# zkh2018/ethsnarks

Measured on AMD Instinct MI355X. Metric: groth16_proofs_per_sec, higher is better.
Workload: dtype u32 (8-limb 254-bit Montgomery integers)

## Files before the change

ethsnarks_amd/csrc/ntt.hpp:

```cpp
#pragma once
#include "bn254.hpp"
#include "common.hpp"

namespace zk {

#ifndef ZK_NTT_TILE_LOG
#define ZK_NTT_TILE_LOG 11
#endif
constexpr int NTT_TILE_LOG = ZK_NTT_TILE_LOG;
constexpr int NTT_TILE = 1 << NTT_TILE_LOG;
#ifndef ZK_NTT_THREADS
#define ZK_NTT_THREADS 512
#endif
constexpr int NTT_THREADS = ZK_NTT_THREADS;
constexpr int NTT_MIN_LOGC = 2;

static ZK_HD uint32_t bitrev32(uint32_t v, uint32_t bits) {
#if defined(__clang__)
    return bits ? __builtin_bitreverse32(v) >> (32 - bits) : 0;
#else
    uint32_t r = 0;
    for (uint32_t i = 0; i < bits; i++) { r = (r << 1) | (v & 1); v >>= 1; }
    return r;
#endif
}

struct NttFuse { const fe *in2 = nullptr; const fe *post_alt = nullptr; uint32_t alt_from = 0xffffffffu; const fe *sub = nullptr; };
__global__ void __launch_bounds__(NTT_THREADS)
k_ntt_pass(const fe *__restrict__ in, fe *__restrict__ out, const fe *__restrict__ tw,
           uint32_t logm, uint32_t s0, uint32_t k, uint32_t logc, int bitrev_load,
           const fe *__restrict__ pre, const fe *__restrict__ post, uint32_t batch_stride, NttFuse fuse, int last_pass) {
    __shared__ uint32_t sh[8][NTT_TILE];
    in += (size_t)blockIdx.y * batch_stride; out += (size_t)blockIdx.y * batch_stride;
    if (fuse.in2) fuse.in2 += (size_t)blockIdx.y * batch_stride;
    if (fuse.sub) fuse.sub += (size_t)blockIdx.y * batch_stride;
    if (fuse.post_alt && blockIdx.y >= fuse.alt_from) post = fuse.post_alt;
    const uint32_t tile = 1u << (k + logc), ncol = 1u << logc;
    const uint32_t nlb = (1u << s0) >> logc;
    const uint32_t lb = blockIdx.x & (nlb - 1), h = blockIdx.x / nlb;
    const uint32_t base = (h << (s0 + k)) | (lb << logc);

    auto gidx = [&](uint32_t e) -> uint32_t { return base | ((e >> logc) << s0) | (e & (ncol - 1)); };
    auto fetch = [&](uint32_t idx) -> fe {
        const uint32_t src = bitrev_load ? bitrev32(idx, logm) : idx;
        fe v = in[src];
        if (fuse.in2) v = Fr::mul(v, fuse.in2[src]);
        if (pre) v = Fr::mul(v, pre[src]);
        return v;
    };
    auto emit = [&](uint32_t idx, fe v) {
        if (post) v = Fr::mul(v, post[idx]);
        else if (last_pass) v = Fr::canon(v);
        if (fuse.sub) v = Fr::sub(v, fuse.sub[idx]);
        out[idx] = v;
    };
    const bool load_fused = k >= 2;
    if (!load_fused) {
        for (uint32_t e = threadIdx.x; e < tile; e += blockDim.x) {
            const fe v = fetch(gidx(e));
#pragma unroll
            for (int l = 0; l < 8; l++) sh[l][e] = v.l[l];
        }
        __syncthreads();
    }
    uint32_t s = 1;
    for (; s + 1 <= k; s += 2) {
        const uint32_t half = 1u << (s - 1), S = s0 + s;
        const bool from_mem = s == 1, to_mem = s + 1 == k;
        for (uint32_t qd = threadIdx.x; qd < (tile >> 2); qd += blockDim.x) {
            const uint32_t c = qd & (ncol - 1), r = qd >> logc;
            const uint32_t jm = r & (half - 1), grp = r >> (s - 1);
            const uint32_t e00 = (((grp << (s + 1)) | jm) << logc) | c, e01 = e00 + (half << logc), e10 = e00 + (half << (logc + 1)), e11 = e10 + (half << logc);
            const uint32_t j = (jm << s0) | ((lb << logc) | c);
            const size_t i2 = (size_t)j << (logm - S - 1);
            fe x0, x1, x2, x3;
            if (from_mem) { x0 = fetch(gidx(e00)); x1 = fetch(gidx(e01)); x2 = fetch(gidx(e10)); x3 = fetch(gidx(e11)); }
            else {
#pragma unroll
                for (int l = 0; l < 8; l++) { x0.l[l] = sh[l][e00]; x1.l[l] = sh[l][e01]; x2.l[l] = sh[l][e10]; x3.l[l] = sh[l][e11]; }
            }
#ifdef ZK_NTT_NOPAIR
            if (S > 1) { const fe t1 = tw[i2 << 1]; x1 = Fr::lmul(x1, t1); x3 = Fr::lmul(x3, t1); }
#else
            if (S > 1) { const fe t1 = tw[i2 << 1]; Fr::lmul_pair(x1, t1, x3, t1, x1, x3); }
#endif
            fe a0 = Fr::ladd(x0, x1), a1 = Fr::lsub(x0, x1), a2 = Fr::ladd(x2, x3), a3 = Fr::lsub(x2, x3);
            if (S == 1) a3 = Fr::lmul(a3, tw[(size_t)1 << (logm - 2)]);
            else {
#ifdef ZK_NTT_NOPAIR
                a2 = Fr::lmul(a2, tw[i2]); a3 = Fr::lmul(a3, tw[i2 + ((size_t)1 << (logm - 2))]);
#else
                Fr::lmul_pair(a2, tw[i2], a3, tw[i2 + ((size_t)1 << (logm - 2))], a2, a3);
#endif
            }
            x0 = Fr::ladd(a0, a2); x2 = Fr::lsub(a0, a2); x1 = Fr::ladd(a1, a3); x3 = Fr::lsub(a1, a3);
            if (to_mem) { emit(gidx(e00), x0); emit(gidx(e01), x1); emit(gidx(e10), x2); emit(gidx(e11), x3); }
            else {
#pragma unroll
                for (int l = 0; l < 8; l++) { sh[l][e00] = x0.l[l]; sh[l][e01] = x1.l[l]; sh[l][e10] = x2.l[l]; sh[l][e11] = x3.l[l]; }
            }
        }
        if (!to_mem) __syncthreads();
    }
    if (s <= k) {
        const uint32_t half = 1u << (s - 1), S = s0 + s;
        for (uint32_t bf = threadIdx.x; bf < (tile >> 1); bf += blockDim.x) {
            uint32_t c = bf & (ncol - 1), q = bf >> logc;
            uint32_t jm = q & (half - 1), grp = q >> (s - 1);
            uint32_t eu = (((grp << s) | jm) << logc) | c, ev = eu + (half << logc);
            uint32_t j = (jm << s0) | ((lb << logc) | c);
            fe u, v;
#pragma unroll
            for (int l = 0; l < 8; l++) { u.l[l] = sh[l][eu]; v.l[l] = sh[l][ev]; }
            if (S > 1) v = Fr::lmul(v, tw[(size_t)j << (logm - S)]);
            emit(gidx(eu), Fr::ladd(u, v)); emit(gidx(ev), Fr::lsub(u, v));
        }
    } else if (k == 0) {
        for (uint32_t e = threadIdx.x; e < tile; e += blockDim.x) {
            fe v;
#pragma unroll
            for (int l = 0; l < 8; l++) v.l[l] = sh[l][e];
            emit(gidx(e), v);
        }
    }
}

__global__ void k_fill_geometric(fe *out, uint32_t n, fe g, fe s) {
    uint32_t run = blockIdx.x * blockDim.x + threadIdx.x;
    uint32_t i0 = run * 256;
// ... 18 lines not shown
static inline fe fr_domain_root(uint32_t logm) {
    fe w; const uint32_t c[8] = {0x725b19f0u, 0x9bd61b6eu, 0x41112ed4u, 0x402d111eu, 0x8ef62abcu, 0x00e0a7ebu, 0xa58a7e85u, 0x2a3c09f0u};
    for (int i = 0; i < 8; i++) w.l[i] = c[i];
    w = Fr::to_mont(w);
    for (uint32_t i = logm; i < 28; i++) w = Fr::sqr(w);
    return w;
}

static inline int ntt_tables_free(NttTables &t) {
    if (t.tw_fwd) hipFree(t.tw_fwd);
    if (t.tw_inv) hipFree(t.tw_inv);
    if (t.coset_fwd) hipFree(t.coset_fwd);
    if (t.inv_m) hipFree(t.inv_m);
    if (t.icoset) hipFree(t.icoset);
    if (t.inv_then_coset) hipFree(t.inv_then_coset);
    if (t.inv_m_zinv) hipFree(t.inv_m_zinv);
    if (t.icoset_zinv) hipFree(t.icoset_zinv);
    t = NttTables();
    return ZK_OK;
}

static inline int ntt_tables_create(NttTables &t, uint32_t logm, hipStream_t st) {
    if (logm > 28) return ZK_ERR_ARG;
    t.logm = logm;
    const uint32_t m = 1u << logm, half = m > 1 ? m / 2 : 1;
    ZK_HIP(hipMalloc(&t.tw_fwd, sizeof(fe) * half));
    ZK_HIP(hipMalloc(&t.tw_inv, sizeof(fe) * half));
    ZK_HIP(hipMalloc(&t.coset_fwd, sizeof(fe) * m));
    ZK_HIP(hipMalloc(&t.inv_m, sizeof(fe) * m));
    ZK_HIP(hipMalloc(&t.icoset, sizeof(fe) * m));
    ZK_HIP(hipMalloc(&t.inv_then_coset, sizeof(fe) * m));
    ZK_HIP(hipMalloc(&t.inv_m_zinv, sizeof(fe) * m));
    ZK_HIP(hipMalloc(&t.icoset_zinv, sizeof(fe) * m));
    const fe w = fr_domain_root(logm), wi = Fr::inv(w), g = Fr::from_u64(5), gi = Fr::inv(g);
    const fe mi = Fr::inv(Fr::from_u64(m)), one = Fr::one();
    t.zinv = Fr::inv(Fr::sub(Fr::pow_u64(g, m), one));
    auto fill = [&](fe *dst, uint32_t n, const fe &base, const fe &scale) {
        uint32_t runs = zk_div_up(n, 256);
        ZK_LAUNCH(k_fill_geometric, zk_div_up(runs, 64), 64, st, dst, n, base, scale);
    };
    fill(t.tw_fwd, half, w, one);
    fill(t.tw_inv, half, wi, one);
    fill(t.coset_fwd, m, g, one);
    fill(t.inv_m, m, one, mi);
    fill(t.icoset, m, gi, mi);
    fill(t.inv_then_coset, m, g, mi);
    fill(t.inv_m_zinv, m, one, Fr::mul(mi, t.zinv));
    fill(t.icoset_zinv, m, gi, Fr::mul(mi, t.zinv));
    ZK_HIP(hipGetLastError());
    return ZK_OK;
}

static inline int ntt_run(const NttTables &t, const fe *in, fe *out, bool inverse,
                          const fe *pre, const fe *post, hipStream_t st, uint32_t batch = 1, uint32_t stride = 0, NttFuse fuse = NttFuse()) {
    const uint32_t logm = t.logm, m = 1u << logm;
    const fe *tw = inverse ? t.tw_inv : t.tw_fwd;
    if (logm == 0) {
        uint32_t k0 = 0;
        ZK_LAUNCH_SYNC(k_ntt_pass, dim3(1, batch), NTT_THREADS, st, in, out, tw, logm, 0u, k0, 0u, 1, pre, post, stride, fuse, 1);
        return ZK_OK;
    }
    const uint32_t k0 = logm < (uint32_t)NTT_TILE_LOG ? logm : NTT_TILE_LOG;
    uint32_t rem = logm - k0;
    const uint32_t kmax = NTT_TILE_LOG - NTT_MIN_LOGC;
    uint32_t npass = (rem + kmax - 1) / kmax;
    NttFuse first = fuse, later = fuse;
    later.in2 = nullptr;
    if (rem != 0) { first.post_alt = nullptr; first.sub = nullptr; }
    ZK_LAUNCH_SYNC(k_ntt_pass, dim3(m >> k0, batch), NTT_THREADS, st, in, out, tw, logm, 0u, k0, 0u, 1, pre,
                   rem == 0 ? post : (const fe *)nullptr, stride, first, rem == 0 ? 1 : 0);
    uint32_t s0 = k0;
    while (rem) {
        uint32_t k = (rem + npass - 1) / npass;
        uint32_t logc = NTT_TILE_LOG - k;
        if (logc > s0) logc = s0;
        rem -= k; npass--;
        NttFuse f = later;
        if (rem != 0) { f.post_alt = nullptr; f.sub = nullptr; }
        ZK_LAUNCH_SYNC(k_ntt_pass, dim3(m >> (k + logc), batch), NTT_THREADS, st, (const fe *)out, out, tw, logm, s0, k, logc, 0,
                       (const fe *)nullptr, rem == 0 ? post : (const fe *)nullptr, stride, f, rem == 0 ? 1 : 0);
        s0 += k;
    }
    ZK_HIP(hipGetLastError());
    return ZK_OK;
}

constexpr uint32_t SPMV_LONG_ROW = 64;
constexpr uint32_t SPMV_CHUNK = 4096;

static ZK_HD bool fr_is_one(const fe &a) {
    uint32_t t = 0;
#pragma unroll
    for (int i = 0; i < 8; i++) t |= a.l[i] ^ FrParams::one(i);
    return t == 0;
}
static ZK_D fe spmv_term(const fe &coef, const fe &x) { return fr_is_one(coef) ? x : Fr::mul(coef, x); }

__global__ void k_spmv_rows(const uint32_t *__restrict__ row_ptr, const uint32_t *__restrict__ col,
                            const fe *__restrict__ coeff, const fe *__restrict__ w, fe *__restrict__ out, uint32_t n_rows,
                            uint32_t w_stride, uint32_t out_stride, uint32_t m_rows, uint32_t n_in_rows) {
    uint32_t j = blockIdx.x * blockDim.x + threadIdx.x;
    if (j >= m_rows) return;
    w += (size_t)blockIdx.y * w_stride; out += (size_t)blockIdx.y * out_stride;
    if (j >= n_rows) { out[j] = j - n_rows < n_in_rows ? w[j - n_rows] : Fr::zero(); return; }
    uint32_t b = row_ptr[j], e = row_ptr[j + 1];
    if (e - b > SPMV_LONG_ROW) return;
    fe acc = Fr::zero();
    for (uint32_t k = b; k < e; k++) acc = Fr::add(acc, spmv_term(coeff[k], w[col[k]]));
    out[j] = acc;
}

__global__ void __launch_bounds__(256)
k_spmv_long_chunks(const uint32_t *__restrict__ chunk_begin, const uint32_t *__restrict__ chunk_end,
                   const uint32_t *__restrict__ col, const fe *__restrict__ coeff, const fe *__restrict__ w,
                   fe *__restrict__ partial, uint32_t w_stride) {
    __shared__ uint32_t sh[8][256];
    w += (size_t)blockIdx.y * w_stride; partial += (size_t)blockIdx.y * gridDim.x;
    const uint32_t b = chunk_begin[blockIdx.x], e = chunk_end[blockIdx.x];
    fe acc = Fr::zero();
    for (uint32_t k = b + threadIdx.x; k < e; k += blockDim.x) acc = Fr::add(acc, spmv_term(coeff[k], w[col[k]]));
#pragma unroll
    for (int l = 0; l < 8; l++) sh[l][threadIdx.x] = acc.l[l];
    __syncthreads();
    for (uint32_t s = 128; s > 0; s >>= 1) {
        if (threadIdx.x < s) {
            fe o;
#pragma unroll
            for (int l = 0; l < 8; l++) o.l[l] = sh[l][threadIdx.x + s];
            acc = Fr::add(acc, o);
#pragma unroll
            for (int l = 0; l < 8; l++) sh[l][threadIdx.x] = acc.l[l];
        }
        __syncthreads();
    }
    if (threadIdx.x == 0) partial[blockIdx.x] = acc;
}

__global__ void __launch_bounds__(256)
k_spmv_long_finish(const uint32_t *__restrict__ long_row, const uint32_t *__restrict__ long_first_chunk,
                   const fe *__restrict__ partial, fe *__restrict__ out, uint32_t n_long, uint32_t n_chunks, uint32_t out_stride) {
    __shared__ uint32_t sh[8][256];
    const uint32_t i = blockIdx.x;
    if (i >= n_long) return;
    partial += (size_t)blockIdx.y * n_chunks; out += (size_t)blockIdx.y * out_stride;
    fe acc = Fr::zero();
    for (uint32_t k = long_first_chunk[i] + threadIdx.x; k < long_first_chunk[i + 1]; k += blockDim.x) acc = Fr::add(acc, partial[k]);
#pragma unroll
    for (int l = 0; l < 8; l++) sh[l][threadIdx.x] = acc.l[l];
    __syncthreads();
// ... 16 lines not shown
```

ethsnarks_amd/csrc/zkhip.cpp:

```cpp
#include <algorithm>
#include <atomic>
#include <memory>
#include <mutex>
#include <new>
#include <stdexcept>
#include <string>
#include <vector>
#include <chrono>
#include <string.h>
#include <stddef.h>
#include <stdlib.h>
#include <sys/stat.h>

#include "common.hpp"
#include "bn254.hpp"
#include "ntt.hpp"
#include "msm.hpp"
#include "keygen.hpp"
#include "blind.hpp"
#include "../../include/zkhip.h"
#include <errno.h>
#include <sys/random.h>

namespace zk { thread_local char g_last_error[256] = ""; }
// ... 448 lines not shown
    return full_save(path, codec, k);
} ZK_GUARD
extern "C" int zk_pk_is_full(const zk_pk *pk) try { return pk && pk->full ? 1 : 0; } ZK_GUARD

namespace {
struct DevCsr {
    uint32_t n_rows = 0, nnz = 0, n_long = 0, n_chunks = 0;
    uint32_t *row_ptr = nullptr, *col = nullptr, *long_row = nullptr, *long_first = nullptr, *chunk_begin = nullptr, *chunk_end = nullptr;
    fe *coeff = nullptr, *partial = nullptr;
    void release() {
        void *p[] = {row_ptr, col, long_row, long_first, chunk_begin, chunk_end, coeff, partial};
        for (void *q : p) if (q) hipFree(q);
        *this = DevCsr();
    }
    int upload(const zk_csr *m, uint32_t V, uint32_t batch) {
        n_rows = m->n_rows;
        nnz = m->row_ptr[n_rows];
        std::vector<uint32_t> lrow, lfirst, cb, ce;
        for (uint32_t j = 0; j < n_rows; j++) {
            uint32_t b = m->row_ptr[j], e = m->row_ptr[j + 1];
            if (e < b || e > nnz) return fail(ZK_ERR_ARG, "CSR row_ptr not monotone");
            if (e - b > SPMV_LONG_ROW) {
                lrow.push_back(j); lfirst.push_back((uint32_t)cb.size());
                for (uint32_t k = b; k < e; k += SPMV_CHUNK) { cb.push_back(k); ce.push_back(k + SPMV_CHUNK < e ? k + SPMV_CHUNK : e); }
            }
        }
        lfirst.push_back((uint32_t)cb.size());
        for (uint32_t k = 0; k < nnz; k++) if (m->col[k] > V) return fail(ZK_ERR_ARG, "CSR column index exceeds the number of variables");
        n_long = (uint32_t)lrow.size(); n_chunks = (uint32_t)cb.size();
        ZK_HIP(hipMalloc(&row_ptr, 4 * (size_t)(n_rows + 1)));
        ZK_HIP(hipMalloc(&col, 4 * (size_t)(nnz + 1)));
        ZK_HIP(hipMalloc(&coeff, 32 * (size_t)(nnz + 1)));
        ZK_HIP(hipMemcpy(row_ptr, m->row_ptr, 4 * (size_t)(n_rows + 1), hipMemcpyHostToDevice));
        if (nnz) {
            ZK_HIP(hipMemcpy(col, m->col, 4 * (size_t)nnz, hipMemcpyHostToDevice));
            ZK_HIP(hipMemcpy(coeff, m->coeff, 32 * (size_t)nnz, hipMemcpyHostToDevice));
        }
        ZK_HIP(hipMalloc(&long_row, 4 * (size_t)(n_long + 1)));
        ZK_HIP(hipMalloc(&long_first, 4 * (size_t)(n_long + 1)));
        ZK_HIP(hipMalloc(&chunk_begin, 4 * (size_t)(n_chunks + 1)));
        ZK_HIP(hipMalloc(&chunk_end, 4 * (size_t)(n_chunks + 1)));
        ZK_HIP(hipMalloc(&partial, 32 * ((size_t)n_chunks * batch + 1)));
        if (n_long) ZK_HIP(hipMemcpy(long_row, lrow.data(), 4 * (size_t)n_long, hipMemcpyHostToDevice));
        ZK_HIP(hipMemcpy(long_first, lfirst.data(), 4 * (size_t)(n_long + 1), hipMemcpyHostToDevice));
        if (n_chunks) {
            ZK_HIP(hipMemcpy(chunk_begin, cb.data(), 4 * (size_t)n_chunks, hipMemcpyHostToDevice));
            ZK_HIP(hipMemcpy(chunk_end, ce.data(), 4 * (size_t)n_chunks, hipMemcpyHostToDevice));
        }
        return ZK_OK;
    }
    int enqueue(const fe *w, fe *out, hipStream_t st, uint32_t batch, uint32_t w_stride, uint32_t out_stride, uint32_t m_rows = 0, uint32_t n_in_rows = 0) const {
        if (m_rows < n_rows) m_rows = n_rows;
        if (m_rows) ZK_LAUNCH(k_spmv_rows, dim3(zk_div_up(m_rows, 256), batch), 256, st, (const uint32_t *)row_ptr, (const uint32_t *)col, (const fe *)coeff, w, out, n_rows, w_stride, out_stride, m_rows, n_in_rows);
        if (n_chunks) {
            ZK_LAUNCH_SYNC(k_spmv_long_chunks, dim3(n_chunks, batch), 256, st, (const uint32_t *)chunk_begin, (const uint32_t *)chunk_end,
                           (const uint32_t *)col, (const fe *)coeff, w, partial, w_stride);
            ZK_LAUNCH_SYNC(k_spmv_long_finish, dim3(n_long, batch), 256, st, (const uint32_t *)long_row, (const uint32_t *)long_first,
                      (const fe *)partial, out, n_long, n_chunks, out_stride);
        }
        ZK_HIP(hipGetLastError());
        return ZK_OK;
    }
};

__global__ void k_to_mont(fe *a, uint32_t n) {
    uint32_t i = blockIdx.x * blockDim.x + threadIdx.x;
    if (i < n) a[i] = Fr::to_mont(a[i]);
}
__global__ void k_field_mul(const fe *a, const fe *b, fe *o, uint32_t n, int field) {
    uint32_t i = blockIdx.x * blockDim.x + threadIdx.x;
    if (i < n) o[i] = field ? Fq::mul(a[i], b[i]) : Fr::mul(a[i], b[i]);
}

template <class T> int dev_upload(T **dst, const T *src, size_t n) {
    ZK_HIP(hipMalloc(dst, sizeof(T) * (n ? n : 1)));
    if (n) ZK_HIP(hipMemcpy(*dst, src, sizeof(T) * n, hipMemcpyHostToDevice));
    return ZK_OK;
}
struct Range { uint32_t lo, hi; uint32_t n() const { return hi - lo; } };
Range shard_range(uint32_t n, uint32_t rank, uint32_t count) {
    return Range{(uint32_t)((uint64_t)n * rank / count), (uint32_t)((uint64_t)n * (rank + 1) / count)};
}
}


namespace {
struct DeviceTables {
    uint64_t pk_id = 0; int device = 0; uint32_t rank = 0, count = 1, cbits = 0;
    uint32_t max_batch = 1;
    uint32_t cA = 0, cB = 0, cH = 0, cL = 0;
    G1::Affine *tA = nullptr, *tH = nullptr, *tL = nullptr; G2::Affine *tB = nullptr;
    uint32_t *dA_idx = nullptr, *dB_idx = nullptr;
    bool zk = false;
    G1::Affine *tB1 = nullptr, *tD1 = nullptr; G2::Affine *tD2 = nullptr;
    bool share_A = false, share_B = false, share_L = false;
    uint32_t win_lo = 0, win_n = 0;
    uint32_t *posA = nullptr, *posB = nullptr;
    uint32_t offA = 0, offB = 0, offL = 0;
    uint32_t cW = 0;
    uint32_t plog = 0;
    uint64_t table_bytes = 0, full_table_bytes = 0;
    bool key_alive = true;
    int refs = 0;
    void free_device() {
        DeviceScope on(device);
        void *dev[] = {tA, tH, tL, tB, dA_idx, dB_idx, posA, posB, tB1, tD1, tD2};
// ... 64 lines not shown
}
void stream_park(hipStream_t st, int device, int role, int prio) {
    if (!st) return;
    (void)hipStreamSynchronize(st);
    std::lock_guard<std::mutex> lk(g_streams_mu);
    g_streams.push_back(ParkedStream{device, role, prio, st});
}
enum { ROLE_MAIN = 0, ROLE_ACC, ROLE_A, ROLE_B, ROLE_L, ROLE_COPY };
}

namespace { std::atomic<int> g_dev_inflight[64]; }
struct zk_ctx {
    int device = 0;
    int stream_prio[6] = {0, 0, 0, 0, 0, 0};
    DeviceTables *tables = nullptr;
    bool serial = false;
    bool in_flight = false;
    bool alone_hint = false;
    void set_in_flight(bool on) {
        if (on != in_flight && device >= 0 && device < 64) g_dev_inflight[device].fetch_add(on ? 1 : -1, std::memory_order_relaxed);
        in_flight = on;
    }
    bool awaiting_h = false;
    uint32_t max_batch = 1, cur_batch = 1;
    uint32_t nC = 0, nIn = 0, V = 0, m = 0, logm = 0;
    zk_config cfg{};
    G1::Affine alpha_g1; G2::Affine beta_g2;
    Range rA{}, rB{}, rH{}, rL{};
    uint32_t *dA_idx = nullptr, *dB_idx = nullptr;
    DevCsr cA, cB, cC;
    fe *d_w = nullptr, *d_a = nullptr, *d_b = nullptr, *d_c = nullptr, *d_t = nullptr;
    uint8_t *d_partials = nullptr;
    fe *h_w = nullptr;
    fe *d_w2 = nullptr, *h_w2 = nullptr;
    hipStream_t s_copy = nullptr;
    hipEvent_t ev_staged = nullptr;
    uint32_t staged_k = 0; int staged_canonical = 0;
    fe *h_tail = nullptr;
    NttTables tab;
    MsmWork<G1> mA, mH, mL, mW; MsmWork<G2> mB;
    MsmWork<G1> mB1;
    uint8_t *d_zk = nullptr, *h_zk = nullptr;
    G1::Affine beta_g1;
    bool cur_zk = false;
    hipEvent_t ev_z1 = nullptr, ev_z2 = nullptr, ev_zf = nullptr;
    hipStream_t s_main = nullptr, s_acc = nullptr, s_a = nullptr, s_b = nullptr, s_l = nullptr;
    hipStream_t s_h = nullptr;
    hipEvent_t ev_up = nullptr, ev_sort_h = nullptr;
    bool h_stream_made = false;
    bool latency_call = false;
    bool merge_hl = false;
    bool cur_merge = false;
    bool env_no_direct_h2d = false;
    int env_h_stream = -1;
    char env_h_borrow = 0;
    char env_hl_tail = 0;
    int env_b_tail_lanes = 0;
    bool env_tails_on_acc = false;
    hipEvent_t ev_sort = nullptr;
    hipEvent_t ev_start = nullptr, ev_w = nullptr, ev_h = nullptr, ev_a0 = nullptr, ev_a1 = nullptr, ev_b0 = nullptr, ev_b1 = nullptr,
               ev_l0 = nullptr, ev_l1 = nullptr, ev_h1 = nullptr, ev_h0 = nullptr;
    ~zk_ctx() {
        set_in_flight(false);
        DeviceScope on(device);
        void *dev[] = {d_w, d_a, d_t, d_partials};
        for (void *p : dev) if (p) hipFree(p);
        if (h_w) hipHostFree(h_w);
        if (d_w2) hipFree(d_w2);
        if (h_w2) hipHostFree(h_w2);
        stream_park(s_copy, device, ROLE_COPY, stream_prio[ROLE_COPY]);
        if (ev_staged) hipEventDestroy(ev_staged);
        if (h_tail) hipHostFree(h_tail);
        cA.release(); cB.release(); cC.release();
        ntt_tables_free(tab);
        mA.release(); mH.release(); mL.release(); mB.release(); mW.release(); mB1.release();
        if (d_zk) hipFree(d_zk);
        if (ev_z1) hipEventDestroy(ev_z1);
        if (ev_z2) hipEventDestroy(ev_z2);
        if (ev_zf) hipEventDestroy(ev_zf);
        if (h_zk) { memset(h_zk, 0, (BLIND_RS_BYTES + BLIND_G1_BYTES + BLIND_G2_BYTES) * max_batch); hipHostFree(h_zk); }
        tables_release(tables);
        if (serial) s_a = s_b = s_l = nullptr;
        if (s_acc == s_main) s_acc = nullptr;
        if (ev_sort) hipEventDestroy(ev_sort);
        s_h = nullptr;
        if (ev_up) hipEventDestroy(ev_up);
        if (ev_sort_h) hipEventDestroy(ev_sort_h);
        stream_park(s_main, device, ROLE_MAIN, stream_prio[ROLE_MAIN]); stream_park(s_acc, device, ROLE_ACC, stream_prio[ROLE_ACC]);
        stream_park(s_a, device, ROLE_A, stream_prio[ROLE_A]); stream_park(s_b, device, ROLE_B, stream_prio[ROLE_B]); stream_park(s_l, device, ROLE_L, stream_prio[ROLE_L]);
        hipEvent_t ee[] = {ev_start, ev_w, ev_h, ev_a0, ev_a1, ev_b0, ev_b1, ev_l0, ev_l1, ev_h1, ev_h0};
        for (auto e : ee) if (e) hipEventDestroy(e);
    }
};

extern "C" uint32_t zk_domain_size(uint32_t nC, uint32_t nIn) {
    uint32_t v = nC + nIn + 1;
    v--; v |= v >> 1; v |= v >> 2; v |= v >> 4; v |= v >> 8; v |= v >> 16; v++;
    return v;
}

static int ctx_build(zk_ctx *c, const zk_pk *pk, const zk_csr *A, const zk_csr *B, const zk_csr *C) {
    ZK_TRY(use_device(c->device));
    const uint32_t m = c->m, V = c->V, nIn = c->nIn;
    const uint32_t G = c->cfg.shard_count > 1 ? c->cfg.shard_count : 1, r = G > 1 ? c->cfg.shard_rank : 0;
    c->rA = shard_range((uint32_t)pk->a_val.size(), r, G);
    c->rB = shard_range((uint32_t)pk->b_val.size(), r, G);
// ... 71 lines not shown
                if (rc == ZK_OK) { blind_table_host<G1>(pk->delta_g1, d1); rc = dev_upload(&t->tD1, d1.data(), d1.size()); }
                if (rc == ZK_OK) { blind_table_host<G2>(pk->delta_g2, d2); rc = dev_upload(&t->tD2, d2.data(), d2.size()); }
            }
            if (rc != ZK_OK) return rc;
            g_tables.push_back(t);
            fresh.release();
        }
        t->refs++;
        c->tables = t;
    }
    c->dA_idx = c->tables->dA_idx; c->dB_idx = c->tables->dB_idx;
    const DeviceTables *t = c->tables;
    const bool any_share = t->share_A || t->share_B || t->share_L;
    const uint32_t KB = c->max_batch;
    if (any_share) { ZK_TRY(c->mW.alloc(t->win_n, t->cW, nullptr, nullptr, true, KB, t->plog)); c->mW.use_shift_payload(); }
    ZK_TRY(c->mA.alloc(c->rA.n(), t->cA, t->tA, t->share_A ? &c->mW.sh : nullptr, false, KB, t->plog));
    ZK_TRY(c->mH.alloc(c->rH.n(), t->cH, t->tH, nullptr, false, KB, t->plog));
    ZK_TRY(c->mL.alloc(c->rL.n(), t->cL, t->tL, t->share_L ? &c->mW.sh : nullptr, false, KB, t->plog));
    ZK_TRY(c->mB.alloc(c->rB.n(), t->cB, t->tB, t->share_B ? &c->mW.sh : nullptr, false, KB, t->plog));
    if (t->zk) {
        ZK_TRY(c->mB1.alloc(c->rB.n(), t->cB, t->tB1, t->share_B ? &c->mW.sh : &c->mB.sh, false, KB, t->plog));
        const size_t per = BLIND_RS_BYTES + BLIND_G1_BYTES + BLIND_G2_BYTES;
        ZK_HIP(hipMalloc(&c->d_zk, (per + BLIND_FIX_BYTES) * KB));
        ZK_HIP(hipHostMalloc(&c->h_zk, per * KB, hipHostMallocDefault));
        memset(c->h_zk, 0, per * KB);
        ZK_HIP(hipEventCreate(&c->ev_z1)); ZK_HIP(hipEventCreate(&c->ev_z2));
        ZK_HIP(hipEventCreateWithFlags(&c->ev_zf, hipEventDisableTiming));
        c->beta_g1 = pk->beta_g1;
    }
    ZK_TRY(c->cA.upload(A, V, KB)); ZK_TRY(c->cB.upload(B, V, KB)); ZK_TRY(c->cC.upload(C, V, KB));
    ZK_HIP(hipMalloc(&c->d_w, 32 * (size_t)(V + 1) * KB));
    ZK_HIP(hipMalloc(&c->d_a, 3 * 32 * (size_t)m * KB)); c->d_b = c->d_a + (size_t)m * KB; c->d_c = c->d_a + 2 * (size_t)m * KB;
    ZK_HIP(hipMalloc(&c->d_t, 3 * 32 * (size_t)m * KB));
    ZK_HIP(hipMalloc(&c->d_partials, sizeof(zk_partials) * KB));
    ZK_HIP(hipMemset(c->d_partials, 0, sizeof(zk_partials) * KB));
    c->merge_hl = c->rH.n() && c->rL.n() && c->mH.sh.nb == c->mL.sh.nb && c->mH.sh.plog == c->mL.sh.plog && !getenv("ZK_NO_MERGE_HL");
    if (G > 1) {
        c->mA.dev_result = (G1::XYZZ *)(c->d_partials + offsetof(zk_partials, At)); c->mB.dev_result = (G2::XYZZ *)(c->d_partials + offsetof(zk_partials, Bt));
        c->mH.dev_result = (G1::XYZZ *)(c->d_partials + offsetof(zk_partials, Ht));
        if (!c->merge_hl) c->mL.dev_result = (G1::XYZZ *)(c->d_partials + offsetof(zk_partials, Lt));
    }
    c->mA.dev_result_pitch = c->mB.dev_result_pitch = c->mH.dev_result_pitch = c->mL.dev_result_pitch = sizeof(zk_partials);
    ZK_HIP(hipHostMalloc(&c->h_w, 32 * (size_t)(V + 1) * KB, hipHostMallocDefault));
    ZK_HIP(hipHostMalloc(&c->h_tail, 32 * (size_t)KB, hipHostMallocDefault));
    int prio_lo = 0, prio_hi = 0;
    ZK_HIP(hipDeviceGetStreamPriorityRange(&prio_lo, &prio_hi));
    const bool latency_sched = c->cfg.schedule == ZK_SCHED_LATENCY && (uint64_t)c->mH.sh.max_entries() * c->max_batch >= (3ull << 18);
    const char *pr = getenv("ZK_PRIOS");
    if (!pr || strlen(pr) != 5) pr = latency_sched ? "hhhhh" : "hllhl";
    auto prio = [&](char ch) { return ch == 'h' ? prio_hi : ch == 'l' ? prio_lo : (prio_hi + prio_lo) / 2; };
    for (int i = 0; i < 5; i++) c->stream_prio[i] = prio(pr[i]);
    ZK_TRY(stream_take(&c->s_main, c->device, ROLE_MAIN, c->stream_prio[ROLE_MAIN]));
    c->env_no_direct_h2d = getenv("ZK_NO_DIRECT_H2D") != nullptr;
    if (const char *e = getenv("ZK_H_STREAM")) c->env_h_stream = e[0] == '1' ? 1 : 0;
    if (const char *e = getenv("ZK_H_BORROW")) c->env_h_borrow = e[0];
    if (const char *e = getenv("ZK_HL_TAIL")) c->env_hl_tail = e[0];
    if (const char *e = getenv("ZK_B_TAIL_LANES")) c->env_b_tail_lanes = atoi(e);
    c->env_tails_on_acc = getenv("ZK_TAILS_ON_ACC") != nullptr;
    const char *serial = getenv("ZK_SERIAL");
    c->serial = (serial && serial[0] == '1') || c->cfg.schedule == ZK_SCHED_ONE_STREAM;
    const char *split = getenv("ZK_SPLIT_STREAMS");
    if (c->serial || (split && split[0] == '0')) c->s_acc = c->s_main;
    else ZK_TRY(stream_take(&c->s_acc, c->device, ROLE_ACC, c->stream_prio[ROLE_ACC]));
    ZK_HIP(hipEventCreate(&c->ev_sort));
    c->s_h = c->s_main;
    if (c->serial) { c->s_a = c->s_b = c->s_l = c->s_main; }
    else {
        ZK_TRY(stream_take(&c->s_a, c->device, ROLE_A, c->stream_prio[ROLE_A]));
        ZK_TRY(stream_take(&c->s_b, c->device, ROLE_B, c->stream_prio[ROLE_B]));
        ZK_TRY(stream_take(&c->s_l, c->device, ROLE_L, c->stream_prio[ROLE_L]));
    }
    hipEvent_t *ee[] = {&c->ev_start, &c->ev_w, &c->ev_h, &c->ev_a0, &c->ev_a1, &c->ev_b0, &c->ev_b1, &c->ev_l0, &c->ev_l1, &c->ev_h1, &c->ev_h0};
    for (auto e : ee) ZK_HIP(hipEventCreate(e));
    ZK_TRY(ntt_tables_create(c->tab, c->logm, c->s_main));
    ZK_HIP(hipStreamSynchronize(c->s_main));
    return ZK_OK;
}

extern "C" int zk_ctx_create(const zk_pk *pk, const zk_csr *A, const zk_csr *B, const zk_csr *C,
                             uint32_t nC, uint32_t nIn, uint32_t V, const zk_config *cfg, zk_ctx **out) try {
    if (!pk || !A || !B || !C || !out) return fail(ZK_ERR_ARG, "null argument");
    if (A->n_rows != nC || B->n_rows != nC || C->n_rows != nC) return fail(ZK_ERR_ARG, "CSR row counts must equal nC");
    if (nIn > V) return fail(ZK_ERR_ARG, "nIn > V");
    if ((uint64_t)nC + nIn + 1 > (1ull << 28)) return fail(ZK_ERR_ARG, "domain exceeds 2^28 (2-adicity of r - 1)");
    const uint32_t m = zk_domain_size(nC, nIn);
    if (pk->a_domain != V + 1 || pk->b_domain != V + 1 || pk->H.size() != (size_t)m - 1 || pk->L.size() != (size_t)(V - nIn))
        return fail(ZK_ERR_SHAPE, "proving key shape does not match (A/B domain = V+1, |H| = m-1, |L| = V-nIn)");
    std::unique_ptr<zk_ctx> holder(new zk_ctx());
    zk_ctx *c = holder.get();
    if (cfg) c->cfg = *cfg;
    if (c->cfg.shard_count > 1 && c->cfg.shard_rank >= c->cfg.shard_count) return fail(ZK_ERR_ARG, "shard_rank >= shard_count");
    c->device = (int)c->cfg.device;
    c->max_batch = c->cfg.max_batch ? c->cfg.max_batch : 1;
    if (c->max_batch > 4096) return fail(ZK_ERR_ARG, "max_batch > 4096");
    c->nC = nC; c->nIn = nIn; c->V = V; c->m = m;
    while ((1u << c->logm) < m) c->logm++;
    c->alpha_g1 = pk->alpha_g1; c->beta_g2 = pk->beta_g2;
    ZK_TRY(ctx_build(c, pk, A, B, C));
    *out = holder.release();
    return ZK_OK;
} ZK_GUARD
extern "C" int zk_ctx_create_sized(const zk_pk *pk, const zk_csr *A, const zk_csr *B, const zk_csr *C,
                                   uint32_t nC, uint32_t nIn, uint32_t V, const zk_config *cfg, size_t cfg_size, zk_ctx **out) try {
    zk_config full{};
    if (cfg) memcpy(&full, cfg, cfg_size < sizeof(full) ? cfg_size : sizeof(full));
    return zk_ctx_create(pk, A, B, C, nC, nIn, V, cfg ? &full : nullptr, out);
} ZK_GUARD
extern "C" void zk_ctx_destroy(zk_ctx *ctx) try { delete ctx; } ZK_GUARD_VOID

static int enqueue_compute_h(zk_ctx *c, hipStream_t st) {
    const uint32_t m = c->m, k = c->cur_batch, ws = c->V + 1;
    fe *a = c->d_a, *b = c->d_a + (size_t)m * k, *cc = c->d_a + 2 * (size_t)m * k;
    ZK_TRY(c->cA.enqueue(c->d_w, a, st, k, ws, m, m, c->nIn + 1));
    ZK_TRY(c->cB.enqueue(c->d_w, b, st, k, ws, m, m, 0));
    ZK_TRY(c->cC.enqueue(c->d_w, cc, st, k, ws, m, m, 0));
    (void)cc;
    NttFuse cscale; cscale.post_alt = c->tab.inv_m_zinv; cscale.alt_from = 2 * k;
    ZK_TRY(ntt_run(c->tab, a, c->d_t, true, nullptr, c->tab.inv_then_coset, st, 3 * k, m, cscale));
    ZK_TRY(ntt_run(c->tab, c->d_t, a, false, nullptr, nullptr, st, 2 * k, m));
    NttFuse last; last.in2 = b; last.sub = c->d_t + 2 * (size_t)m * k;
    ZK_TRY(ntt_run(c->tab, a, c->d_t, true, nullptr, c->tab.icoset_zinv, st, k, m, last));
    if (k == 1) ZK_HIP(hipMemcpyAsync(c->h_tail, c->d_t + (m - 1), 32, hipMemcpyDeviceToHost, st));
    else ZK_HIP(hipMemcpy2DAsync(c->h_tail, 32, c->d_t + (m - 1), 32 * (size_t)m, 32, k, hipMemcpyDeviceToHost, st));
    ZK_HIP(hipGetLastError());
    return ZK_OK;
}

static int enqueue_chain(zk_ctx *c, int which) {
    hipStream_t st = c->s_main;
    const uint32_t m = c->m, ws = c->V + 1;
    fe *p = c->d_a + (size_t)which * m, *tmp = c->d_t + (size_t)which * m;
    const DevCsr &M = which == 0 ? c->cA : which == 1 ? c->cB : c->cC;
    ZK_TRY(M.enqueue(c->d_w, p, st, 1, ws, m, m, which == 0 ? c->nIn + 1 : 0));
    if (which == 2) return ntt_run(c->tab, p, tmp, true, nullptr, c->tab.inv_m_zinv, st);
    ZK_TRY(ntt_run(c->tab, p, tmp, true, nullptr, c->tab.inv_then_coset, st));
    ZK_TRY(ntt_run(c->tab, tmp, p, false, nullptr, nullptr, st));
    return ZK_OK;
}
static int enqueue_h_from_chains(zk_ctx *c, const fe *a, const fe *b, const fe *cc) {
    hipStream_t st = c->s_main;
    const uint32_t m = c->m;
    if (cc >= c->d_t && cc < c->d_t + m) return fail(ZK_ERR_ARG, "zk_h_from_chains_submit: the C chain overlaps the context's h buffer");
    NttFuse last; last.in2 = b; last.sub = cc;
    ZK_TRY(ntt_run(c->tab, a, c->d_t, true, nullptr, c->tab.icoset_zinv, st, 1, m, last));
    ZK_HIP(hipMemcpyAsync(c->h_tail, c->d_t + (m - 1), 32, hipMemcpyDeviceToHost, st));
    return ZK_OK;
}

static int upload_witness(zk_ctx *c, const uint64_t *witness, int canonical, int resident = 0) {
    const size_t n = (size_t)(c->V + 1) * c->cur_batch;
    const bool direct = resident == 3 || (!resident && c->latency_call && !c->env_no_direct_h2d);
    if (resident == 3) resident = 0;
    if (!resident && !direct) memcpy(c->h_w, witness, 32 * n);
    if (resident == 2) ZK_HIP(hipStreamWaitEvent(c->s_main, c->ev_staged, 0));
    ZK_HIP(hipEventRecord(c->ev_start, c->s_main));
    if (resident == 1) ZK_HIP(hipMemcpyAsync(c->d_w, witness, 32 * n, hipMemcpyDeviceToDevice, c->s_main));
    else if (direct) ZK_HIP(hipMemcpyAsync(c->d_w, witness, 32 * n, hipMemcpyHostToDevice, c->s_main));
    else if (!resident) ZK_HIP(hipMemcpyAsync(c->d_w, c->h_w, 32 * n, hipMemcpyHostToDevice, c->s_main));
    if (canonical) ZK_LAUNCH(k_to_mont, zk_div_up(n, 256), 256, c->s_main, c->d_w, (uint32_t)n);
    ZK_HIP(hipEventRecord(c->ev_w, c->s_main));
    return ZK_OK;
}

static void store_xyzz(uint64_t *dst, const G1::XYZZ &p) { memcpy(dst, &p, sizeof(p)); }
static void store_xyzz(uint64_t *dst, const G2::XYZZ &p) { memcpy(dst, &p, sizeof(p)); }

enum { PHASE_ALL = 0, PHASE_WITNESS = 1, PHASE_H = 2 };
static int prove_enqueue(zk_ctx *c, const uint64_t *witness, int canonical, int resident, const fe *d_h, int phase);
static void zk_clear_rs(zk_ctx *c);
static void drain(zk_ctx *c) {
    c->mL.tail_pending = c->mH.tail_pending = c->mB1.tail_pending = false;
// ... 989 lines not shown
```

Baseline: 116.0.

## Fuse short-row sparse matrix-vector products into the first inverse NTT pass load

The A/B/C constraint-matrix SpMV for short rows is now computed inside the first pass of the batched inverse NTT, at the bit-reversed load, instead of in a separate kernel that writes the polynomial to memory. Long rows are still handled by the chunked kernel ahead of time, and the fused load picks up their precomputed value. This removes one full write and read of the 3×batch polynomial buffers and a kernel launch. In exchange the NTT load stage becomes irregular and branchy, with scattered witness reads, which can raise register pressure and cause lane divergence in the NTT kernel.

```diff
diff --git a/ethsnarks_amd/csrc/ntt.hpp b/ethsnarks_amd/csrc/ntt.hpp
--- a/ethsnarks_amd/csrc/ntt.hpp
+++ b/ethsnarks_amd/csrc/ntt.hpp
@@ -26,10 +26,61 @@
 }
 
 struct NttFuse { const fe *in2 = nullptr; const fe *post_alt = nullptr; uint32_t alt_from = 0xffffffffu; const fe *sub = nullptr; };
+constexpr uint32_t SPMV_LONG_ROW = 64;
+struct NttRows {
+    const uint32_t *row_ptr[3] = {nullptr, nullptr, nullptr}, *col[3] = {nullptr, nullptr, nullptr};
+    const fe *coeff[3] = {nullptr, nullptr, nullptr};
+    const fe *w = nullptr;
+    uint32_t w_stride = 0, n_rows = 0, k = 1, n_in_rows = 0;
+};
+static ZK_HD bool fr_is_one(const fe &a) {
+    uint32_t t = 0;
+#pragma unroll
+    for (int i = 0; i < 8; i++) t |= a.l[i] ^ FrParams::one(i);
+    return t == 0;
+}
+static ZK_D fe spmv_term(const fe &coef, const fe &x) { return fr_is_one(coef) ? x : Fr::mul(coef, x); }
+static ZK_D void ntt_rows_fetch4(const NttRows &R, const fe *__restrict__ in, const uint32_t src[4], fe v[4]) {
+    const uint32_t mat = blockIdx.y / R.k, p = blockIdx.y - mat * R.k;
+    const uint32_t *__restrict__ row_ptr = mat == 0 ? R.row_ptr[0] : mat == 1 ? R.row_ptr[1] : R.row_ptr[2];
+    const uint32_t *__restrict__ col = mat == 0 ? R.col[0] : mat == 1 ? R.col[1] : R.col[2];
+    const fe *__restrict__ coeff = mat == 0 ? R.coeff[0] : mat == 1 ? R.coeff[1] : R.coeff[2];
+    const uint32_t n_in = mat == 0 ? R.n_in_rows : 0;
+    const fe *__restrict__ w = R.w + (size_t)p * R.w_stride;
+    uint32_t b[4], e[4];
+#pragma unroll
+    for (int u = 0; u < 4; u++) {
+        b[u] = e[u] = 0;
+        if (src[u] < R.n_rows) { b[u] = row_ptr[src[u]]; e[u] = row_ptr[src[u] + 1]; }
+    }
+#pragma unroll
+    for (int u = 0; u < 4; u++) {
+        const uint32_t j = src[u];
+        if (j >= R.n_rows) v[u] = j - R.n_rows < n_in ? w[j - R.n_rows] : Fr::zero();
+        else if (e[u] - b[u] > SPMV_LONG_ROW) { v[u] = in[j]; e[u] = b[u]; }
+        else v[u] = Fr::zero();
+    }
+    for (uint32_t t = 0;; t++) {
+        bool any = false;
+        uint32_t cl[4];
+#pragma unroll
+        for (int u = 0; u < 4; u++) if (b[u] + t < e[u]) { cl[u] = col[b[u] + t]; any = true; }
+        if (!any) break;
+#pragma unroll
+        for (int h = 0; h < 4; h += 2) {
+            fe cf[2], x[2];
+#pragma unroll
+            for (int u = 0; u < 2; u++) if (b[h + u] + t < e[h + u]) { cf[u] = coeff[b[h + u] + t]; x[u] = w[cl[h + u]]; }
+#pragma unroll
+            for (int u = 0; u < 2; u++) if (b[h + u] + t < e[h + u]) v[h + u] = Fr::add(v[h + u], spmv_term(cf[u], x[u]));
+        }
+    }
+}
+template <bool ROWS>
 __global__ void __launch_bounds__(NTT_THREADS)
 k_ntt_pass(const fe *__restrict__ in, fe *__restrict__ out, const fe *__restrict__ tw,
            uint32_t logm, uint32_t s0, uint32_t k, uint32_t logc, int bitrev_load,
-           const fe *__restrict__ pre, const fe *__restrict__ post, uint32_t batch_stride, NttFuse fuse, int last_pass) {
+           const fe *__restrict__ pre, const fe *__restrict__ post, uint32_t batch_stride, NttFuse fuse, int last_pass, NttRows rows) {
     __shared__ uint32_t sh[8][NTT_TILE];
     in += (size_t)blockIdx.y * batch_stride; out += (size_t)blockIdx.y * batch_stride;
     if (fuse.in2) fuse.in2 += (size_t)blockIdx.y * batch_stride;
@@ -47,6 +98,14 @@
         if (fuse.in2) v = Fr::mul(v, fuse.in2[src]);
         if (pre) v = Fr::mul(v, pre[src]);
         return v;
+    };
+    auto fetch4 = [&](uint32_t i0, uint32_t i1, uint32_t i2, uint32_t i3, fe &x0, fe &x1, fe &x2, fe &x3) {
+        if constexpr (ROWS) {
+            const uint32_t src[4] = {bitrev32(i0, logm), bitrev32(i1, logm), bitrev32(i2, logm), bitrev32(i3, logm)};
+            fe v[4];
+            ntt_rows_fetch4(rows, in, src, v);
+            x0 = v[0]; x1 = v[1]; x2 = v[2]; x3 = v[3];
+        } else { x0 = fetch(i0); x1 = fetch(i1); x2 = fetch(i2); x3 = fetch(i3); }
     };
     auto emit = [&](uint32_t idx, fe v) {
         if (post) v = Fr::mul(v, post[idx]);
@@ -74,7 +133,7 @@
             const uint32_t j = (jm << s0) | ((lb << logc) | c);
             const size_t i2 = (size_t)j << (logm - S - 1);
             fe x0, x1, x2, x3;
-            if (from_mem) { x0 = fetch(gidx(e00)); x1 = fetch(gidx(e01)); x2 = fetch(gidx(e10)); x3 = fetch(gidx(e11)); }
+            if (from_mem) fetch4(gidx(e00), gidx(e01), gidx(e10), gidx(e11), x0, x1, x2, x3);
             else {
 #pragma unroll
                 for (int l = 0; l < 8; l++) { x0.l[l] = sh[l][e00]; x1.l[l] = sh[l][e01]; x2.l[l] = sh[l][e10]; x3.l[l] = sh[l][e11]; }
@@ -199,23 +258,30 @@
 }
 
 static inline int ntt_run(const NttTables &t, const fe *in, fe *out, bool inverse,
-                          const fe *pre, const fe *post, hipStream_t st, uint32_t batch = 1, uint32_t stride = 0, NttFuse fuse = NttFuse()) {
+                          const fe *pre, const fe *post, hipStream_t st, uint32_t batch = 1, uint32_t stride = 0, NttFuse fuse = NttFuse(),
+                          const NttRows *rows = nullptr) {
     const uint32_t logm = t.logm, m = 1u << logm;
     const fe *tw = inverse ? t.tw_inv : t.tw_fwd;
     if (logm == 0) {
         uint32_t k0 = 0;
-        ZK_LAUNCH_SYNC(k_ntt_pass, dim3(1, batch), NTT_THREADS, st, in, out, tw, logm, 0u, k0, 0u, 1, pre, post, stride, fuse, 1);
+        if (rows) return ZK_ERR_ARG;
+        ZK_LAUNCH_SYNC(k_ntt_pass<false>, dim3(1, batch), NTT_THREADS, st, in, out, tw, logm, 0u, k0, 0u, 1, pre, post, stride, fuse, 1, NttRows());
         return ZK_OK;
     }
     const uint32_t k0 = logm < (uint32_t)NTT_TILE_LOG ? logm : NTT_TILE_LOG;
+    if (rows && (k0 < 2 || fuse.in2 || pre)) return ZK_ERR_ARG;
     uint32_t rem = logm - k0;
     const uint32_t kmax = NTT_TILE_LOG - NTT_MIN_LOGC;
     uint32_t npass = (rem + kmax - 1) / kmax;
     NttFuse first = fuse, later = fuse;
     later.in2 = nullptr;
     if (rem != 0) { first.post_alt = nullptr; first.sub = nullptr; }
-    ZK_LAUNCH_SYNC(k_ntt_pass, dim3(m >> k0, batch), NTT_THREADS, st, in, out, tw, logm, 0u, k0, 0u, 1, pre,
-                   rem == 0 ? post : (const fe *)nullptr, stride, first, rem == 0 ? 1 : 0);
+    if (rows)
+        ZK_LAUNCH_SYNC(k_ntt_pass<true>, dim3(m >> k0, batch), NTT_THREADS, st, in, out, tw, logm, 0u, k0, 0u, 1, pre,
+                       rem == 0 ? post : (const fe *)nullptr, stride, first, rem == 0 ? 1 : 0, *rows);
+    else
+        ZK_LAUNCH_SYNC(k_ntt_pass<false>, dim3(m >> k0, batch), NTT_THREADS, st, in, out, tw, logm, 0u, k0, 0u, 1, pre,
+                       rem == 0 ? post : (const fe *)nullptr, stride, first, rem == 0 ? 1 : 0, NttRows());
     uint32_t s0 = k0;
     while (rem) {
         uint32_t k = (rem + npass - 1) / npass;
@@ -224,24 +290,15 @@
         rem -= k; npass--;
         NttFuse f = later;
         if (rem != 0) { f.post_alt = nullptr; f.sub = nullptr; }
-        ZK_LAUNCH_SYNC(k_ntt_pass, dim3(m >> (k + logc), batch), NTT_THREADS, st, (const fe *)out, out, tw, logm, s0, k, logc, 0,
-                       (const fe *)nullptr, rem == 0 ? post : (const fe *)nullptr, stride, f, rem == 0 ? 1 : 0);
+        ZK_LAUNCH_SYNC(k_ntt_pass<false>, dim3(m >> (k + logc), batch), NTT_THREADS, st, (const fe *)out, out, tw, logm, s0, k, logc, 0,
+                       (const fe *)nullptr, rem == 0 ? post : (const fe *)nullptr, stride, f, rem == 0 ? 1 : 0, NttRows());
         s0 += k;
     }
     ZK_HIP(hipGetLastError());
     return ZK_OK;
 }
 
-constexpr uint32_t SPMV_LONG_ROW = 64;
 constexpr uint32_t SPMV_CHUNK = 4096;
-
-static ZK_HD bool fr_is_one(const fe &a) {
-    uint32_t t = 0;
-#pragma unroll
-    for (int i = 0; i < 8; i++) t |= a.l[i] ^ FrParams::one(i);
-    return t == 0;
-}
-static ZK_D fe spmv_term(const fe &coef, const fe &x) { return fr_is_one(coef) ? x : Fr::mul(coef, x); }
 
 __global__ void k_spmv_rows(const uint32_t *__restrict__ row_ptr, const uint32_t *__restrict__ col,
                             const fe *__restrict__ coeff, const fe *__restrict__ w, fe *__restrict__ out, uint32_t n_rows,
diff --git a/ethsnarks_amd/csrc/zkhip.cpp b/ethsnarks_amd/csrc/zkhip.cpp
--- a/ethsnarks_amd/csrc/zkhip.cpp
+++ b/ethsnarks_amd/csrc/zkhip.cpp
@@ -524,6 +524,9 @@
     int enqueue(const fe *w, fe *out, hipStream_t st, uint32_t batch, uint32_t w_stride, uint32_t out_stride, uint32_t m_rows = 0, uint32_t n_in_rows = 0) const {
         if (m_rows < n_rows) m_rows = n_rows;
         if (m_rows) ZK_LAUNCH(k_spmv_rows, dim3(zk_div_up(m_rows, 256), batch), 256, st, (const uint32_t *)row_ptr, (const uint32_t *)col, (const fe *)coeff, w, out, n_rows, w_stride, out_stride, m_rows, n_in_rows);
+        return enqueue_long(w, out, st, batch, w_stride, out_stride);
+    }
+    int enqueue_long(const fe *w, fe *out, hipStream_t st, uint32_t batch, uint32_t w_stride, uint32_t out_stride) const {
         if (n_chunks) {
             ZK_LAUNCH_SYNC(k_spmv_long_chunks, dim3(n_chunks, batch), 256, st, (const uint32_t *)chunk_begin, (const uint32_t *)chunk_end,
                            (const uint32_t *)col, (const fe *)coeff, w, partial, w_stride);
@@ -694,6 +697,7 @@
     bool merge_hl = false;
     bool cur_merge = false;
     bool env_no_direct_h2d = false;
+    bool env_no_fused_rows = false;
     int env_h_stream = -1;
     char env_h_borrow = 0;
     char env_hl_tail = 0;
@@ -871,6 +875,7 @@
     for (int i = 0; i < 5; i++) c->stream_prio[i] = prio(pr[i]);
     ZK_TRY(stream_take(&c->s_main, c->device, ROLE_MAIN, c->stream_prio[ROLE_MAIN]));
     c->env_no_direct_h2d = getenv("ZK_NO_DIRECT_H2D") != nullptr;
+    c->env_no_fused_rows = getenv("ZK_NO_FUSED_ROWS") != nullptr;
     if (const char *e = getenv("ZK_H_STREAM")) c->env_h_stream = e[0] == '1' ? 1 : 0;
     if (const char *e = getenv("ZK_H_BORROW")) c->env_h_borrow = e[0];
     if (const char *e = getenv("ZK_HL_TAIL")) c->env_hl_tail = e[0];
@@ -930,12 +935,24 @@
 static int enqueue_compute_h(zk_ctx *c, hipStream_t st) {
     const uint32_t m = c->m, k = c->cur_batch, ws = c->V + 1;
     fe *a = c->d_a, *b = c->d_a + (size_t)m * k, *cc = c->d_a + 2 * (size_t)m * k;
-    ZK_TRY(c->cA.enqueue(c->d_w, a, st, k, ws, m, m, c->nIn + 1));
-    ZK_TRY(c->cB.enqueue(c->d_w, b, st, k, ws, m, m, 0));
-    ZK_TRY(c->cC.enqueue(c->d_w, cc, st, k, ws, m, m, 0));
+    const bool fused = !c->env_no_fused_rows && c->logm >= 2;
+    NttRows rows;
+    if (fused) {
+        const DevCsr *M[3] = {&c->cA, &c->cB, &c->cC};
+        for (int i = 0; i < 3; i++) { rows.row_ptr[i] = M[i]->row_ptr; rows.col[i] = M[i]->col; rows.coeff[i] = M[i]->coeff; }
+        rows.w = c->d_w; rows.w_stride = ws; rows.n_rows = c->nC; rows.k = k; rows.n_in_rows = c->nIn + 1;
+        ZK_TRY(c->cA.enqueue_long(c->d_w, a, st, k, ws, m));
+        ZK_TRY(c->cB.enqueue_long(c->d_w, b, st, k, ws, m));
+        ZK_TRY(c->cC.enqueue_long(c->d_w, cc, st, k, ws, m));
+    } else {
+        ZK_TRY(c->cA.enqueue(c->d_w, a, st, k, ws, m, m, c->nIn + 1));
+        ZK_TRY(c->cB.enqueue(c->d_w, b, st, k, ws, m, m, 0));
+        ZK_TRY(c->cC.enqueue(c->d_w, cc, st, k, ws, m, m, 0));
+    }
     (void)cc;
     NttFuse cscale; cscale.post_alt = c->tab.inv_m_zinv; cscale.alt_from = 2 * k;
-    ZK_TRY(ntt_run(c->tab, a, c->d_t, true, nullptr, c->tab.inv_then_coset, st, 3 * k, m, cscale));
+    ZK_TRY(ntt_run(c->tab, a, c->d_t, true, nullptr, c->tab.inv_then_coset, st, 3 * k, m, cscale,
+                   fused ? &rows : nullptr));
     ZK_TRY(ntt_run(c->tab, c->d_t, a, false, nullptr, nullptr, st, 2 * k, m));
     NttFuse last; last.in2 = b; last.sub = c->d_t + 2 * (size_t)m * k;
     ZK_TRY(ntt_run(c->tab, a, c->d_t, true, nullptr, c->tab.icoset_zinv, st, k, m, last));
```

Result: no change. 116.2 (median of 6 runs) (+0.1%).
